# ShenhanQian/KGDet

Measured on AMD Instinct MI355X. Metric: training images/sec (whole node) KGDet R50-FPN 800x1333, higher is better.
Workload: dtype f32 (3 MFMA products per multiply on hi/lo-split operands -- fp16 parts forward, bf16 parts for gradients --, f32 accumulate); 1 GPU; KGDet R50-FPN train step, 2 img/GPU at 800x1333 (padded 800x1344), DeformConv fwd/bwd + focal/moment losses + grad-clip + Adam; no collective at dp1 (one rank: nothing to exchange); global_batch=2, parallelism=dp1

## Files before the change

### include/kgdet_hip.h

```cpp
#ifndef KGDET_HIP_H_
#define KGDET_HIP_H_

#include <stddef.h>
#include <stdint.h>

#ifdef __cplusplus
extern "C" {
#endif

#define KGDET_OK 0
#define KGDET_E_SHAPE 1
#define KGDET_E_WORKSPACE 2
#define KGDET_E_HIP 3
size_t kgdet_conv_packed_bytes(int32_t M, int32_t K, int32_t taps);
int kgdet_conv_pack(const float *w, int32_t O, int32_t C, int32_t taps, int32_t transpose, void *packed, void *stream);
int kgdet_conv_pack_fmt(const float *w, int32_t O, int32_t C, int32_t taps, int32_t transpose, void *packed,
                        int32_t operand_format, void *stream);
int kgdet_conv_pack_both_fmt(const float *w, int32_t O, int32_t C, int32_t taps, void *packed, void *packed_t,
                             int32_t forward_format, void *stream);
int kgdet_conv_apply_epilogue_fmt(const void *packed, const float *x, float *y, const float *bias, const float *residual,
                                  int32_t relu, int64_t B, int32_t M, int32_t K, int32_t H, int32_t W, int32_t taps,
                                  int32_t stride, int32_t operand_format, void *workspace, size_t workspace_bytes,
                                  void *stream);
int kgdet_conv_apply_gated_fmt(const void *packed, const float *x, float *y, const float *bias, const float *residual,
                               int32_t relu, const float *gate, int64_t B, int32_t M, int32_t K, int32_t H, int32_t W,
                               int32_t taps, int32_t stride, int32_t operand_format, void *workspace, size_t workspace_bytes,
                               void *stream);
int kgdet_stem_conv7x7_s2_fmt(const void *packed, const float *x, float *y, int64_t B, int32_t H, int32_t W,
                              int32_t operand_format, void *stream);
int kgdet_conv_pack_both(const float *w, int32_t O, int32_t C, int32_t taps, void *packed, void *packed_t, void *stream);
int64_t kgdet_conv_pack_blocks(int32_t O, int32_t C, int32_t taps);
int kgdet_conv_pack_multi(const int64_t *desc_dev, int32_t n, int64_t total_blocks, void *stream);
size_t kgdet_conv_apply_workspace_bytes(int64_t B, int32_t M, int32_t K, int32_t H, int32_t W, int32_t taps,
                                        int32_t stride);
int kgdet_conv_apply(const void *packed, const float *x, float *y, int64_t B, int32_t M, int32_t K, int32_t H, int32_t W,
                     int32_t taps, int32_t stride, void *workspace, size_t workspace_bytes, void *stream);
#define KGDET_CONV_APPLY_PLAN_WORDS 11
int kgdet_conv_apply_plan(int64_t B, int32_t M, int32_t K, int32_t H, int32_t W, int32_t taps, int32_t stride,
                          int32_t out[KGDET_CONV_APPLY_PLAN_WORDS]);
int kgdet_conv_apply_epilogue(const void *packed, const float *x, float *y, const float *bias, const float *residual,
                              int32_t relu, int64_t B, int32_t M, int32_t K, int32_t H, int32_t W, int32_t taps,
                              int32_t stride, void *workspace, size_t workspace_bytes, void *stream);
int kgdet_stem_conv7x7_s2(const void *packed, const float *x, float *y, int64_t B, int32_t H, int32_t W, void *stream);
int kgdet_conv3x3_s2_grad_input(const void *packed_t, const float *grad_y, float *grad_x, int64_t B, int32_t C, int32_t O,
                                int32_t Hin, int32_t Win, void *stream);
size_t kgdet_conv3x3_s2_grad_weight_workspace_bytes(int64_t B, int32_t O, int32_t C, int32_t H, int32_t W);
int kgdet_conv3x3_s2_grad_weight(const float *grad_y, const float *x, float *grad_w, int64_t B, int32_t O, int32_t C, int32_t H,
                                 int32_t W, void *workspace, size_t workspace_bytes, void *stream);
size_t kgdet_conv1x1_grad_weight_workspace_bytes(int64_t B, int32_t O, int32_t C, int64_t HW);
int kgdet_conv1x1_grad_weight(const float *grad_y, const float *x, float *grad_w, int64_t B, int32_t O, int32_t C,
                              int64_t HW, void *workspace, size_t workspace_bytes, void *stream);
size_t kgdet_conv3x3_grad_weight_workspace_bytes(int64_t B, int32_t O, int32_t C, int32_t H, int32_t W);
int kgdet_conv3x3_grad_weight(const float *grad_y, const float *x, float *grad_w, int64_t B, int32_t O, int32_t C,
                              int32_t H, int32_t W, void *workspace, size_t workspace_bytes, void *stream);
#define KGDET_CONV_GRAD_WEIGHT_PLAN_WORDS 10
int kgdet_conv_grad_weight_plan(int64_t B, int32_t O, int32_t C, int32_t H, int64_t W, int32_t taps,
                                int32_t out[KGDET_CONV_GRAD_WEIGHT_PLAN_WORDS]);

int kgdet_bn_act_forward(const float *x, const float *gamma, const float *beta, const float *mean, const float *var,
                         float eps, const float *residual, float *y, int64_t N, int32_t C, int64_t HW, int32_t relu,
                         void *stream);
int32_t kgdet_bn_act_partials(int64_t N, int32_t C, int64_t HW);
int kgdet_bn_act_backward(const float *grad_y, const float *x, const float *y, const float *gamma, const float *beta,
                          const float *mean, const float *var, float eps, int32_t has_residual, int32_t relu,
                          float *grad_x, float *grad_residual, float *partial, float *sums, int64_t N, int32_t C,
                          int64_t HW, void *stream);
int kgdet_conv1x1_nhwc_residual(const void *x, const void *weight, const float *bias, const void *residual, void *out,
                                int64_t M, int32_t K, int32_t N, int32_t relu, void *stream);
int kgdet_conv1x1_nhwc_residual_in(const void *x, const float *in_bias, const void *weight, const float *bias,
                                   const void *residual, void *out, int64_t M, int32_t K, int32_t N, int32_t relu,
                                   void *stream);
int kgdet_bn_fold_backward(const float *grad_z, const float *z, int32_t relu, float *g, float *partial, int64_t N, int32_t C,
                           int64_t HW, void *stream);
int kgdet_bn_fold_finish(const float *partial, int32_t P, const float *w, float *G , const float *s,
                         const float *mean, const float *var, float eps, float *grad_beta ,
                         float *grad_gamma , int32_t O, int32_t CK, void *stream);
int kgdet_conv1x1_grad_weight_fold(const float *grad_y, const float *x, float *grad_w, int64_t B, int32_t O, int32_t C,
                                   int64_t HW, void *workspace, size_t workspace_bytes, const float *w, const float *s,
                                   const float *mean, const float *var, float eps, const float *bn_partial, int32_t P,
                                   float *grad_beta , float *grad_gamma , void *stream);
int kgdet_conv3x3_grad_weight_fold(const float *grad_y, const float *x, float *grad_w, int64_t B, int32_t O, int32_t C,
                                   int32_t H, int32_t W, void *workspace, size_t workspace_bytes, const float *w,
                                   const float *s, const float *mean, const float *var, float eps, const float *bn_partial,
                                   int32_t P, float *grad_beta , float *grad_gamma , void *stream);
int kgdet_bn_relu_maxpool(const float *x, const float *gamma, const float *beta, const float *mean, const float *var,
                          float eps, float *y, int64_t N, int32_t C, int32_t H, int32_t W, void *stream);

int kgdet_bias_act(void *x, const float *bias, const void *residual, int64_t N, int32_t C, int64_t HW, int32_t dtype,
                   int32_t relu, int32_t channels_last, void *stream);
int kgdet_bias_relu_maxpool_nhwc(const void *x, const float *bias, void *y, int64_t N, int32_t C, int32_t H, int32_t W,
                                 int32_t dtype, void *stream);

#define KGDET_E_UNSUPPORTED 4
#define KGDET_E_PARTIAL 5

const char *kgdet_last_error(void);
int kgdet_version(void);
int kgdet_device_cu_count(void);

#define KGDET_OPT_EXACT_BACKWARD 0
#define KGDET_OPT_FWD_COLUMN_WAVE 1
#define KGDET_OPT_WGRAD_STREAMK 2
#define KGDET_OPT_BWD_PHASE 3
#define KGDET_OPT_COUNT 4
int kgdet_set_option(int32_t option, int32_t value);

typedef struct kgdet_dcn_shape {
  int32_t N, C, H, W;
  int32_t O, kh, kw;
  int32_t stride_h, stride_w, pad_h, pad_w, dil_h, dil_w;
  int32_t groups, deformable_groups;
  int32_t out_channel_offset, out_channels_total;
} kgdet_dcn_shape;

#define KGDET_DCN_RELU 1u
#define KGDET_DCN_BF16 2u
#define KGDET_DCN_EXACT_FP32 4u

int kgdet_dcn_output_size(const kgdet_dcn_shape *s, int32_t *Ho, int32_t *Wo);

size_t kgdet_dcn_packed_weight_bytes(const kgdet_dcn_shape *s);
size_t kgdet_dcn_workspace_bytes(const kgdet_dcn_shape *s);

int kgdet_dcn_pack_weight(const kgdet_dcn_shape *s, const float *weight, float *packed, void *stream);
int kgdet_dcn_pack_weight_multi(int32_t n, const kgdet_dcn_shape *const *shapes, const float *const *weights,
                                float *const *packeds, void *stream);
int kgdet_dcn_pack_weight_images(int32_t n, const kgdet_dcn_shape *const *shapes, const float *const *weights,
                                 float *const *packeds, uint32_t images, void *stream);
int32_t kgdet_dcn_split_path_complete(const kgdet_dcn_shape *shape);
int kgdet_dcn_unpack_weight_grad(const kgdet_dcn_shape *s, const float *packed, float *grad_weight,
                                 int accumulate, void *stream);

int kgdet_deform_conv_forward(const kgdet_dcn_shape *s, const float *input, const float *offset,
                              const float *mask , const float *packed_weight,
                              const float *bias , float *output, uint32_t flags,
                              void *workspace, size_t workspace_bytes, void *stream);

size_t kgdet_dcn_group_workspace_bytes(int32_t n, const kgdet_dcn_shape *const *shapes);

int kgdet_deform_conv_forward_grouped(int32_t n, const kgdet_dcn_shape *const *shapes, const float *const *inputs,
                                      const float *const *offsets, const float *const *masks ,
                                      const float *const *packed_weights, const float *const *biases ,
                                      float *const *outputs, uint32_t flags, void *workspace,
                                      size_t workspace_bytes, void *stream);

int kgdet_deform_conv_grad_input(const kgdet_dcn_shape *s, const float *offset, const float *mask ,
                                 const float *packed_weight, const float *grad_output, float *grad_input,
                                 uint32_t flags, void *workspace, size_t workspace_bytes, void *stream);

int kgdet_deform_conv_grad_offset(const kgdet_dcn_shape *s, const float *input, const float *offset,
                                  const float *packed_weight, const float *grad_output, float *grad_offset,
                                  uint32_t flags, void *workspace, size_t workspace_bytes, void *stream);

int kgdet_deform_conv_backward_input_grouped(int32_t n, const kgdet_dcn_shape *const *shapes, const float *const *inputs,
                                             const float *const *offsets, const float *const *packed_weights,
                                             const float *const *grad_outputs, float *const *grad_inputs,
                                             float *const *grad_offsets, void *workspace, size_t workspace_bytes,
                                             void *stream);

int kgdet_deform_conv_grad_weight_grouped(int32_t n, const kgdet_dcn_shape *const *shapes, const float *const *inputs,
                                          const float *const *offsets, const float *const *grad_outputs,
                                          float *const *grad_weights, void *workspace, size_t workspace_bytes,
                                          void *stream);

int kgdet_deform_conv_backward_input(const kgdet_dcn_shape *s, const float *input, const float *offset,
                                     const float *mask , const float *packed_weight,
                                     const float *grad_output, float *grad_input, float *grad_offset,
                                     float *grad_mask , void *workspace,
                                     size_t workspace_bytes, void *stream);

int kgdet_deform_conv_backward_weight(const kgdet_dcn_shape *s, const float *input, const float *offset,
                                      const float *mask , const float *grad_output,
                                      float *grad_weight, float *grad_bias , int accumulate,
                                      void *workspace, size_t workspace_bytes, void *stream);

typedef struct kgdet_psroi_shape {
  int32_t B, C, H, W;
  int32_t R;
  int32_t out_dim, group_size, pooled_size, part_size, sample_per_part;
  int32_t no_trans, num_classes;
  float spatial_scale, trans_std;
} kgdet_psroi_shape;

size_t kgdet_deform_psroi_forward_workspace_bytes(const kgdet_psroi_shape *s);
int kgdet_deform_psroi_forward(const kgdet_psroi_shape *s, const float *data, const float *rois,
                               const float *trans, float *out, float *count, void *workspace, size_t workspace_bytes,
                               void *stream);
// ... 275 lines not shown
```

### kgdet_amd/_lib.py

```python
import ctypes
import os
import subprocess

_HERE = os.path.dirname(os.path.abspath(__file__))
LIB_PATH = os.environ.get('KGDET_LIB') or os.path.join(_HERE, 'libkgdet_hip.so')
CSRC = os.path.join(_HERE, 'csrc')

KGDET_OK = 0
KGDET_E_SHAPE = 1
KGDET_E_WORKSPACE = 2
KGDET_E_HIP = 3
KGDET_E_UNSUPPORTED = 4
KGDET_E_PARTIAL = 5

DCN_RELU = 1
DCN_BF16 = 2
DCN_EXACT_FP32 = 4


class DcnShape(ctypes.Structure):
    _fields_ = [(n, ctypes.c_int32) for n in (
        'N', 'C', 'H', 'W', 'O', 'kh', 'kw', 'stride_h', 'stride_w', 'pad_h', 'pad_w', 'dil_h',
        'dil_w', 'groups', 'deformable_groups', 'out_channel_offset', 'out_channels_total')]


class PsroiShape(ctypes.Structure):
    _fields_ = [(n, ctypes.c_int32) for n in (
        'B', 'C', 'H', 'W', 'R', 'out_dim', 'group_size', 'pooled_size', 'part_size',
        'sample_per_part', 'no_trans', 'num_classes')] + [
        ('spatial_scale', ctypes.c_float), ('trans_std', ctypes.c_float)]


class AugSegment(ctypes.Structure):
    _fields_ = [('boxes', ctypes.c_void_p), ('scores', ctypes.c_void_p), ('kpts', ctypes.c_void_p), ('n', ctypes.c_int64),
                ('img_w', ctypes.c_float), ('scale', ctypes.c_double), ('flip', ctypes.c_int32)]


PREPROC_MAX_JOBS = 32
COCO_ACC_TILE = 1024
COCO_PACK_ROWS = 4
COCO_ORDER_MAX_ROWS = 1024
COCO_ORDER_MAX_LABELS = 64
COCO_JSON_MAX_K = 1024
DRAW_MAX_IMAGES, DRAW_MAX_ROWS, DRAW_MAX_K, DRAW_MAX_LABELS = 32, 1024, 1024, 64


class CocoPackedDets(ctypes.Structure):
    _fields_ = [('n', ctypes.c_int64)] + [(n, ctypes.c_void_p) for n in (
        'cell', 'img_idx', 'cat_idx', 'id', 'score', 'bbox', 'area', 'kxy32')]


class PreprocJob(ctypes.Structure):
    _fields_ = [('src', ctypes.c_void_p), ('src_h', ctypes.c_int32), ('src_w', ctypes.c_int32),
                ('src_row_bytes', ctypes.c_int32), ('dst', ctypes.c_void_p), ('dst_channel_stride', ctypes.c_int64),
                ('dst_row_stride', ctypes.c_int32), ('new_h', ctypes.c_int32), ('new_w', ctypes.c_int32),
                ('out_h', ctypes.c_int32), ('out_w', ctypes.c_int32), ('scale_y', ctypes.c_float),
                ('scale_x', ctypes.c_float), ('flip', ctypes.c_int32)]


PREPROC_AUG_MAX_JOBS = 16
AUG_COLOUR, AUG_BRIGHTNESS, AUG_CONTRAST, AUG_CONTRAST_FIRST, AUG_SATURATION, AUG_HUE, AUG_PERMUTE = 1, 2, 4, 8, 16, 32, 64


class PreprocAugJob(ctypes.Structure):
    _fields_ = PreprocJob._fields_ + [
        ('vh', ctypes.c_int32), ('vw', ctypes.c_int32), ('oy', ctypes.c_int32), ('ox', ctypes.c_int32),
        ('fill', ctypes.c_float * 3), ('delta', ctypes.c_float), ('alpha', ctypes.c_float), ('sat', ctypes.c_float),
        ('hue', ctypes.c_float), ('perm', ctypes.c_int32), ('flags', ctypes.c_uint32)]


def build(force=False):
    cmd = ['make', '-C', CSRC, '-j8']
    if force:
        cmd.append('-B')
    subprocess.check_call(cmd)
    return LIB_PATH


_lib = None


def lib():
    global _lib
    if _lib is None:
        if not os.path.exists(LIB_PATH):
            raise ImportError(
                'kgdet_amd: %s is missing -- run `python -c "import __graft_entry__ as g; g.build()"` '
                'or `make -C kgdet_amd/csrc`. There is no non-HIP fallback.' % LIB_PATH)
        L = ctypes.CDLL(LIB_PATH)
        L.kgdet_last_error.restype = ctypes.c_char_p
        for name in ('kgdet_dcn_packed_weight_bytes', 'kgdet_dcn_workspace_bytes', 'kgdet_dcn_group_workspace_bytes',
                     'kgdet_nms_workspace_bytes', 'kgdet_deform_psroi_backward_workspace_bytes',
                     'kgdet_deform_psroi_forward_workspace_bytes', 'kgdet_head_loss_workspace_bytes', 'kgdet_serial_loss_workspace_bytes',
                     'kgdet_moment_bbox_backward_workspace_bytes', 'kgdet_multiclass_soft_nms_workspace_bytes'):
            if hasattr(L, name):
                getattr(L, name).restype = ctypes.c_size_t
        for name in ('kgdet_multiclass_soft_nms_supported', 'kgdet_multiclass_nms_supported'):
            if hasattr(L, name):
                getattr(L, name).restype = ctypes.c_int
                getattr(L, name).argtypes = [ctypes.c_int32] * 4
        if hasattr(L, 'kgdet_coco_similarity'):
            vp, i32, i64 = ctypes.c_void_p, ctypes.c_int32, ctypes.c_int64
            L.kgdet_coco_similarity.restype = L.kgdet_coco_match.restype = ctypes.c_int
            L.kgdet_coco_similarity.argtypes = [i32, vp, vp, i32, i64, i64, i64] + [vp] * 8 + [i32, vp, vp]
            L.kgdet_coco_match.argtypes = [vp, vp, i32, i64, i64, i64] + [vp] * 6 + [i32, vp, i32] + [vp] * 5
        if hasattr(L, 'kgdet_coco_accumulate'):
            vp, i32, i64 = ctypes.c_void_p, ctypes.c_int32, ctypes.c_int64
            L.kgdet_coco_count_gt.restype = L.kgdet_coco_accumulate.restype = L.kgdet_coco_pack_landmarks.restype = ctypes.c_int
            L.kgdet_coco_count_gt.argtypes = [vp, vp, i64, i32, i32, vp, vp]
            L.kgdet_coco_accumulate.argtypes = [vp] * 9 + [i64] + [i32] * 5 + [i64] + [vp] * 4 + [ctypes.c_size_t, vp]
            L.kgdet_coco_pack_landmarks.argtypes = [vp, i64, i32, i32, vp, vp, vp, vp]
        if hasattr(L, 'kgdet_coco_order_dets'):
            vp, i32, i64 = ctypes.c_void_p, ctypes.c_int32, ctypes.c_int64
            L.kgdet_coco_order_dets.restype = L.kgdet_coco_scatter_dets.restype = ctypes.c_int
            L.kgdet_coco_order_dets.argtypes = [vp, i64, i32, i32, vp, vp, i32, i32, i64, i32, i32, i32] + [vp] * 7
            L.kgdet_coco_scatter_dets.argtypes = ([vp, i64, i32, i32, vp, i32, i64] + [vp] * 5 + [i32, i32]
                                                  + [ctypes.POINTER(CocoPackedDets)] * 2 + [vp, vp])
        if hasattr(L, 'kgdet_coco_json_write'):
            vp, i32, i64 = ctypes.c_void_p, ctypes.c_int32, ctypes.c_int64
            L.kgdet_coco_json_measure.restype = L.kgdet_coco_json_write.restype = ctypes.c_int
            L.kgdet_coco_json_measure.argtypes = [vp, i64, i32, i32] + [vp] * 5 + [i32, i32, vp, vp, vp, i64, vp, vp]
            L.kgdet_coco_json_write.argtypes = [i32, vp, i64, i32, i32] + [vp] * 5 + [i32, i32, i64, i64, i64, vp, i64, vp, vp]
        if hasattr(L, 'kgdet_draw_detections'):
            vp, i32, i64 = ctypes.c_void_p, ctypes.c_int32, ctypes.c_int64
            L.kgdet_draw_detections.restype = ctypes.c_int
            L.kgdet_draw_detections.argtypes = ([vp, i64, vp, i64, vp, vp, i32, vp, i64, i32, i32, vp, i32, vp, vp, i32, vp, vp,
                                                 ctypes.c_float] + [i32] * 6 + [vp])
        _lib = L
    return _lib


def check(rc, what=''):
    if rc == KGDET_OK:
        return
    msg = lib().kgdet_last_error().decode('utf-8', 'replace')
    if rc == KGDET_E_UNSUPPORTED:
        raise NotImplementedError('%s: %s' % (what, msg))
    raise RuntimeError('%s: %s' % (what, msg))


def ptr(t):
    return ctypes.c_void_p(t.data_ptr()) if t is not None else ctypes.c_void_p(0)


def raw_stream(device_index=None):
    import torch
    if device_index is None:
        device_index = torch.cuda.current_device()
    return torch._C._cuda_getCurrentRawStream(device_index)


def current_stream():
    return ctypes.c_void_p(raw_stream())
```

### kgdet_amd/csrc/dense_forward.hip

```cpp
#include "dense_common.h"

namespace kgdet {

__global__ __launch_bounds__(256) void conv1x1_pack(const float *__restrict__ w, int O, int C, int T, int transpose,
                                                    unsigned char *__restrict__ img, unsigned char *__restrict__ img_t,
                                                    int f16_forward) {
  if (gridDim.y == 2) {
    transpose = blockIdx.y;
    img = blockIdx.y ? img_t : img;
  }
  const bool f16 = f16_forward && !transpose;
  f16_saturate_on();
  const int M = transpose ? C : O, K = transpose ? O : C;
  const int k16s = (K + kTK - 1) / kTK;
  const long long total = (long long)((M + kTM - 1) / kTM) * k16s * T * 2 * kTM;
  for (long long i = blockIdx.x * 256LL + threadIdx.x; i < total; i += gridDim.x * 256LL) {
    const int row = (int)(i % kTM);
    const int khalf = (int)((i / kTM) & 1);
    const long long st = i / (2 * kTM);
    const int t = (int)(st % T);
    const int k16 = (int)((st / T) % k16s), mt = (int)(st / ((long long)T * k16s));
    const int m = mt * kTM + row, k0 = k16 * kTK + khalf * 8;
    float v[8];
#pragma unroll
// ... 189 lines not shown
#pragma unroll
    for (int mi = 0; mi < 2; ++mi) {
      acc[mi] = mfma_t<F16>(a[1][mi], bb[0], acc[mi]);
      acc[mi] = mfma_t<F16>(a[0][mi], bb[1], acc[mi]);
      acc[mi] = mfma_t<F16>(a[0][mi], bb[0], acc[mi]);
    }
  };
  {
    Regs R[kPF];
#pragma unroll
    for (int i = 0; i < kPF; ++i) issue(i, R[i]);
    commit(0, R[0]);
    const int full = stages / kPF * kPF;
    for (int s0 = 0; s0 < full; s0 += kPF) {
#pragma unroll
      for (int u = 0; u < kPF; ++u) {
        const int s = s0 + u;
        __syncthreads();
        issue(s + kPF, R[u]);
        multiply(s & 1);
        commit((s + 1) & 1, R[(u + 1) % kPF]);
      }
    }
#pragma unroll
    for (int u = 0; u < kPF - 1; ++u) {
      const int s = full + u;
      if (s < stages) {
        __syncthreads();
        multiply(s & 1);
        if (s + 1 < stages) commit((s + 1) & 1, R[u + 1]);
      }
    }
  }

  float *yb = y + (long long)part * part_stride + (long long)b * M * N;
  const int n = n0 + wn * 32 + (lane & 31);
  if constexpr (F16) {
#pragma unroll
    for (int mi = 0; mi < 2; ++mi)
#pragma unroll
      for (int r = 0; r < 16; ++r) acc[mi][r] *= 1.0f / kF16WeightScale;
  }
  if (bias || residual) {
    const int nc = min(n, N - 1);
    float add[2][16];
#pragma unroll
    for (int mi = 0; mi < 2; ++mi)
#pragma unroll
      for (int r = 0; r < 16; ++r) {
        const int m = min(mt * kTM + wm * 64 + mi * 32 + (r & 3) + 8 * (r >> 2) + 4 * (lane >> 5), M - 1);
        float v = bias ? bias[m] : 0.0f;
        if (residual) v += residual[((long long)b * M + m) * N + nc];
        add[mi][r] = v;
      }
#pragma unroll
    for (int mi = 0; mi < 2; ++mi)
#pragma unroll
      for (int r = 0; r < 16; ++r) acc[mi][r] += add[mi][r];
  }
  if (gate) {
    const int nc = min(n, N - 1);
    float gv[2][16];
#pragma unroll
    for (int mi = 0; mi < 2; ++mi)
#pragma unroll
      for (int r = 0; r < 16; ++r) {
        const int m = min(mt * kTM + wm * 64 + mi * 32 + (r & 3) + 8 * (r >> 2) + 4 * (lane >> 5), M - 1);
        gv[mi][r] = gate[((long long)b * M + m) * N + nc];
      }
#pragma unroll
    for (int mi = 0; mi < 2; ++mi)
#pragma unroll
      for (int r = 0; r < 16; ++r) acc[mi][r] = gv[mi][r] > 0.0f ? acc[mi][r] : 0.0f;
  }
#pragma unroll
  for (int mi = 0; mi < 2; ++mi)
#pragma unroll
    for (int r = 0; r < 16; ++r) {
      const int m = mt * kTM + wm * 64 + mi * 32 + (r & 3) + 8 * (r >> 2) + 4 * (lane >> 5);
      if (m < M && n < N) yb[(long long)m * N + n] = relu ? fmaxf(acc[mi][r], 0.0f) : acc[mi][r];
    }
}

constexpr int kPatchMax = 256;
constexpr int kPatchPart = 2 * kPatchMax * 16;
constexpr int kPatchBuf = 2 * kPatchPart;
template <int WAVES, int NB, bool F16 = false>
__global__ __launch_bounds__(64 * WAVES) void conv3x3_patch4(const unsigned char *__restrict__ img,
                                                             const float *__restrict__ x, float *__restrict__ y, int M,
                                                             int K, int H, int W, int n_mt, int tiles_x, int n_nt,
                                                             int tiles, int ksplit, long long part_stride, int TX, int TY,
                                                             const float *__restrict__ bias,
                                                             const float *__restrict__ residual, int relu,
    const float *__restrict__ gate = nullptr) {
  __shared__ __attribute__((aligned(16))) unsigned char smem[2 * kPatchBuf];
  if constexpr (F16) f16_saturate_on();
  constexpr int HALVES = 4 / WAVES, THREADS = 64 * WAVES, PXT = kPatchMax / THREADS;
  const int unit0 = xcd_tile(blockIdx.x, tiles * ksplit * HALVES);
  if (unit0 >= tiles * ksplit * HALVES) return;
  const int half = unit0 % HALVES, unit = unit0 / HALVES;
  const int part = unit % ksplit, tile = unit / ksplit;
  const int tid = threadIdx.x, lane = tid & 63, wave = (tid >> 6) + half * WAVES;
  const int N = H * W;
  const int chunks_all = K / kTK, per = (chunks_all + ksplit - 1) / ksplit;
  const int c_begin = part * per, c_end = max(c_begin, min(chunks_all, c_begin + per));
  const int chunks = c_end - c_begin, stages = chunks * 9;
  const int mt = tile % n_mt, nt = (tile / n_mt) % n_nt, b = tile / (n_mt * n_nt);
  const int y0 = (nt / tiles_x) * TY, x0 = (nt % tiles_x) * TX;
  const int PW = TX + 2, PP = PW * (TY + 2);

  if (mt * kTM + half * 64 >= M) return;
  bool p_live[PXT];
  int p_off[PXT];
#pragma unroll
  for (int i = 0; i < PXT; ++i) {
    const int pp = tid + i * THREADS;
    const int ppy = pp / PW, ppx = pp - ppy * PW;
    const int iy = y0 - 1 + ppy, ix = x0 - 1 + ppx;
    p_live[i] = pp < PP && iy >= 0 && iy < H && ix >= 0 && ix < W;
    p_off[i] = p_live[i] ? iy * W + ix : 0;
  }
  const float *xb = x + (long long)b * K * N;
  unsigned char *b_dst = smem + tid * 16;

  int b_rd[NB], o_n[NB];
  bool o_live[NB];
#pragma unroll
  for (int nb = 0; nb < NB; ++nb) {
    const int qq = nb * 32 + (lane & 31), q = min(qq, TX * TY - 1);
    const int py = q / TX, px = q - py * TX;
    b_rd[nb] = ((lane >> 5) * kPatchMax + py * PW + px) * 16;
    o_live[nb] = qq < TX * TY && y0 + py < H && x0 + px < W;
    o_n[nb] = o_live[nb] ? (y0 + py) * W + x0 + px : 0;
  }
  const int row_pitch = PW * 16;
  const unsigned char *ag = img + ((long long)mt * chunks_all + min(c_begin, chunks_all - 1)) * 9 * kStage +
                            (lane >> 5) * (kTM * 16) + (wave * 32 + (lane & 31)) * 16;

  f32x16 acc[NB];
#pragma unroll
  for (int i = 0; i < NB; ++i)
#pragma unroll
    for (int r = 0; r < 16; ++r) acc[i][r] = 0.0f;

  float bv[PXT][16];
  auto issue_b = [&](int ci) {
    const float *xp = xb + (long long)min(c_begin + min(ci, chunks - 1), chunks_all - 1) * kTK * N;
#pragma unroll
    for (int i = 0; i < PXT; ++i)
#pragma unroll
      for (int j = 0; j < 16; ++j) bv[i][j] = xp[(long long)j * N + p_off[i]];
  };
  auto commit_b = [&](int buf) {
#pragma unroll
    for (int i = 0; i < PXT; ++i)
#pragma unroll
      for (int j = 0; j < 16; ++j) asm volatile("" : "+v"(bv[i][j]));
#pragma unroll
    for (int i = 0; i < PXT; ++i)
#pragma unroll
      for (int kh = 0; kh < 2; ++kh) {
        float v[8];
#pragma unroll
        for (int j = 0; j < 8; ++j) v[j] = p_live[i] ? bv[i][kh * 8 + j] : 0.0f;
        bf16x8 hi, lo;
        split8_t<F16>(v, hi, lo);
// ... 305 lines not shown
  return ((t0 > t1 ? t0 : t1) + 255) / 256;
}

template <typename Kernel, typename... Args>
void launch_fmt(bool f16, Kernel bf16_kernel, Kernel f16_kernel, unsigned grid, unsigned block, void *stream, Args... args) {
  hipLaunchKernelGGL(f16 ? f16_kernel : bf16_kernel, dim3(grid), dim3(block), 0, (hipStream_t)stream, args...);
}

int nn_ksplit(long long tiles, int stages) {
  if (tiles >= 200) return 1;
  int k = (int)((384 + tiles - 1) / tiles);
  const int most = stages / 8;
  if (k > most) k = most;
  if (k > 8) k = 8;
  return k < 1 ? 1 : k;
}

struct NNPlan {
  bool patch, halves;
  int TX, TY, NB, NW, tiles_x, n_nt, ks;
  long long tiles;
};
NNPlan plan_nn(long long B, int M, int K, int H, int W, int taps, int stride) {
  NNPlan p;
  const int Ho = (H + stride - 1) / stride, Wo = (W + stride - 1) / stride;
  const int n_mt = (M + kTM - 1) / kTM;
  p.patch = taps == 9 && stride == 1;
  p.TX = p.TY = p.tiles_x = 0;
  p.NB = p.NW = 4;
  p.n_nt = (int)(((long long)Ho * Wo + kTN - 1) / kTN);
  if (p.patch) {
    long long best = -1;
    for (int cap = 128; cap <= (M > 64 ? 160 : 128); cap += 32)
      for (int tx = 8; tx <= 126 && tx <= (W + 7) / 8 * 8; ++tx) {
        const int ty = cap / tx;
        if (ty < 1 || (tx + 2) * (ty + 2) > kPatchMax) continue;
        const long long n = (long long)((H + ty - 1) / ty) * ((W + tx - 1) / tx);
        const long long units = n * n_mt * B;
        const long long rounds = units <= 256 ? 256 : units <= 512 ? 512 : units;
        const long long cost = (rounds * (cap / 32)) * 4096 + n * 8 + (cap == 160) * 4 + ((tx + 2) * (ty + 2) > 230);
        if (best < 0 || cost < best) { best = cost; p.TX = tx; p.TY = ty; p.NB = cap / 32; }
      }
    static const int force_tx = env_int("KGDET_CONV_TX", 0);
    if (force_tx > 0 && (force_tx + 2) * (128 / force_tx + 2) <= kPatchMax) { p.TX = force_tx; p.TY = 128 / force_tx; p.NB = 4; }
    p.tiles_x = (W + p.TX - 1) / p.TX;
    p.n_nt = p.tiles_x * ((H + p.TY - 1) / p.TY);
  } else {
    static const int force_nw = env_int("KGDET_CONV_NW", 0);
    const long long hw = (long long)Ho * Wo;
    const long long u4 = (long long)n_mt * ((hw + 127) / 128) * B, u5 = (long long)n_mt * ((hw + 159) / 160) * B;
    const long long c4 = ((u4 + 255) / 256) * 4, c5 = ((u5 + 255) / 256) * 5;
    if (force_nw == 5 || (force_nw == 0 && u4 >= 200 && u5 >= 200 && c5 * 10 <= c4 * 9)) {
      p.NW = 5;
      p.n_nt = (int)((hw + 159) / 160);
    }
  }
  p.tiles = (long long)n_mt * p.n_nt * B;
  p.ks = nn_ksplit(p.tiles, taps * ((K + kTK - 1) / kTK));
  if (p.patch && p.tiles < 200) {
    const int chunks = K / kTK;
    double best = 1e30;
    p.ks = 1;
    for (int ks = 1; ks <= 8 && ks * 2 <= chunks; ++ks) {
      const double out_mb = (double)B * M * Ho * Wo * 4e-6;
      const double cost = (double)((p.tiles * ks + 255) / 256) * ((chunks + ks - 1) / ks) + 0.114 * out_mb * ks;
      if (cost < best) { best = cost; p.ks = ks; }
    }
  }
  static const int force_ks = env_int("KGDET_CONV_KS", 0);
  if (force_ks > 0) p.ks = force_ks;
  static const int force_halves = env_int("KGDET_CONV_HALVES", -1);
  p.halves = p.patch && p.NB == 4 &&
             (force_halves >= 0 ? force_halves != 0 : ((p.ks == 1 && p.tiles > 256 && p.tiles < 400) || M <= 64));
  return p;
}

enum NNCloser { kCloseStore = 0, kCloseSumEpilogue = 1, kCloseSumBiasAct = 2, kCloseSum = 3 };
NNCloser nn_closer(int ks, long long HW, bool epilogue) {
  if (ks <= 1) return kCloseStore;
  if (!epilogue) return kCloseSum;
  return HW % 2 == 0 ? kCloseSumEpilogue : kCloseSumBiasAct;
}

}

}

using namespace kgdet;

extern "C" size_t kgdet_conv_packed_bytes(int32_t M, int32_t K, int32_t taps) {
  if (M <= 0 || K <= 0 || (taps == 9 && K % kTK) || (taps != 1 && taps != 9)) return 0;
  return (size_t)pack_items(M, K, taps) * 32;
}

extern "C" int kgdet_conv_pack_fmt(const float *w, int32_t O, int32_t C, int32_t taps, int32_t transpose, void *packed,
                                   int32_t operand_format, void *stream) {
  const int M = transpose ? C : O, K = transpose ? O : C;
  KGDET_CHECK_SHAPE(taps == 1 || taps == 9, "taps must be 1 (1x1) or 9 (3x3)");
  KGDET_CHECK_SHAPE(O > 0 && C > 0 && (taps == 1 || K % kTK == 0), "reduction length %d is not a multiple of 16", K);
  KGDET_CHECK_SHAPE(w && packed, "null pointer");
  const long long blocks = (pack_items(M, K, taps) + 255) / 256;
  hipLaunchKernelGGL(conv1x1_pack, dim3((unsigned)(blocks > 65535 ? 65535 : blocks)), dim3(256), 0, (hipStream_t)stream, w,
                     O, C, taps, transpose, (unsigned char *)packed, (unsigned char *)nullptr, operand_format == 1 ? 1 : 0);
  KGDET_CHECK_LAUNCH("conv_pack");
  return KGDET_OK;
}

extern "C" int kgdet_conv_pack(const float *w, int32_t O, int32_t C, int32_t taps, int32_t transpose, void *packed,
                               void *stream) {
  return kgdet_conv_pack_fmt(w, O, C, taps, transpose, packed, 0, stream);
}

extern "C" int kgdet_conv_pack_both_fmt(const float *w, int32_t O, int32_t C, int32_t taps, void *packed, void *packed_t,
                                        int32_t forward_format, void *stream) {
  KGDET_CHECK_SHAPE(taps == 1 || taps == 9, "taps must be 1 (1x1) or 9 (3x3)");
  KGDET_CHECK_SHAPE(O > 0 && C > 0 && (taps == 1 || (O % kTK == 0 && C % kTK == 0)), "O and C must be multiples of 16");
  KGDET_CHECK_SHAPE(w && packed && packed_t, "null pointer");
  const long long blocks = pack_both_blocks(O, C, taps);
  hipLaunchKernelGGL(conv1x1_pack, dim3((unsigned)(blocks > 32768 ? 32768 : blocks), 2), dim3(256), 0,
                     (hipStream_t)stream, w, O, C, taps, 0, (unsigned char *)packed, (unsigned char *)packed_t,
                     forward_format == 1 ? 1 : 0);
  KGDET_CHECK_LAUNCH("conv_pack_both");
  return KGDET_OK;
}

extern "C" int kgdet_conv_pack_both(const float *w, int32_t O, int32_t C, int32_t taps, void *packed, void *packed_t,
                                    void *stream) {
  return kgdet_conv_pack_both_fmt(w, O, C, taps, packed, packed_t, 0, stream);
}

extern "C" int64_t kgdet_conv_pack_blocks(int32_t O, int32_t C, int32_t taps) {
  if (O <= 0 || C <= 0 || (taps == 9 && (O % kTK || C % kTK)) || (taps != 1 && taps != 9)) return 0;
  return pack_both_blocks(O, C, taps);
}

extern "C" int kgdet_conv_pack_multi(const int64_t *desc_dev, int32_t n, int64_t total_blocks, void *stream) {
  KGDET_CHECK_SHAPE(desc_dev && n > 0 && total_blocks > 0 && total_blocks < (1LL << 31), "bad descriptor table");
  hipLaunchKernelGGL(conv1x1_pack_multi, dim3((unsigned)total_blocks), dim3(256), 0, (hipStream_t)stream,
                     (const long long *)desc_dev, n);
  KGDET_CHECK_LAUNCH("conv_pack_multi");
  return KGDET_OK;
}

extern "C" size_t kgdet_conv_apply_workspace_bytes(int64_t B, int32_t M, int32_t K, int32_t H, int32_t W,
                                                    int32_t taps, int32_t stride) {
  if (B <= 0 || M <= 0 || K <= 0 || H <= 0 || W <= 0 || (taps == 9 && K % kTK) || stride < 1 || stride > 2) return 0;
  const long long HW = (long long)((H + stride - 1) / stride) * ((W + stride - 1) / stride);
  const int ks = plan_nn(B, M, K, H, W, taps, stride).ks;
  return ks > 1 ? (size_t)ks * B * M * HW * sizeof(float) : 0;
}

extern "C" int kgdet_conv_apply_plan(int64_t B, int32_t M, int32_t K, int32_t H, int32_t W, int32_t taps, int32_t stride,
                                     int32_t out[KGDET_CONV_APPLY_PLAN_WORDS]) {
  KGDET_CHECK_SHAPE(out, "null pointer");
  KGDET_CHECK_SHAPE(B > 0 && M > 0 && K > 0 && H > 0 && W > 0 && (long long)H * W < (1LL << 30), "bad sizes");
  KGDET_CHECK_SHAPE(taps == 1 || taps == 9, "taps must be 1 (1x1) or 9 (3x3)");
  KGDET_CHECK_SHAPE(stride == 1 || stride == 2, "stride must be 1 or 2");
  KGDET_CHECK_SHAPE(taps == 1 || K % kTK == 0, "reduction length %d is not a multiple of 16", K);
  const NNPlan p = plan_nn(B, M, K, H, W, taps, stride);
  KGDET_CHECK_SHAPE(p.tiles < (1LL << 28), "too many tiles");
  const long long HW = (long long)((H + stride - 1) / stride) * ((W + stride - 1) / stride);
  const int32_t words[KGDET_CONV_APPLY_PLAN_WORDS] = {
      p.patch, p.TX, p.TY, p.NB, p.NW, p.ks, p.halves, (int32_t)p.tiles, p.n_nt, nn_closer(p.ks, HW, true), nn_closer(p.ks, HW, false)};
  for (int i = 0; i < KGDET_CONV_APPLY_PLAN_WORDS; ++i) out[i] = words[i];
  return KGDET_OK;
}

extern "C" int kgdet_conv_apply_epilogue_fmt(const void *packed, const float *x, float *y, const float *bias,
                                             const float *residual, int32_t relu, int64_t B, int32_t M, int32_t K,
                                             int32_t H, int32_t W, int32_t taps, int32_t stride, int32_t operand_format,
                                             void *workspace, size_t workspace_bytes, void *stream) {
  return kgdet_conv_apply_gated_fmt(packed, x, y, bias, residual, relu, nullptr, B, M, K, H, W, taps, stride, operand_format,
                                    workspace, workspace_bytes, stream);
}

extern "C" int kgdet_conv_apply_gated_fmt(const void *packed, const float *x, float *y, const float *bias,
                                          const float *residual, int32_t relu, const float *gate, int64_t B, int32_t M,
                                          int32_t K, int32_t H, int32_t W, int32_t taps, int32_t stride,
                                          int32_t operand_format, void *workspace, size_t workspace_bytes, void *stream) {
  const bool f16 = operand_format == 1;
  KGDET_CHECK_SHAPE(B >= 0 && M > 0 && K > 0 && H >= 0 && W >= 0 && (long long)H * W < (1LL << 30), "bad sizes");
  KGDET_CHECK_SHAPE(taps == 1 || taps == 9, "taps must be 1 (1x1) or 9 (3x3)");
  KGDET_CHECK_SHAPE(stride == 1 || stride == 2, "stride must be 1 or 2");
  KGDET_CHECK_SHAPE(taps == 1 || K % kTK == 0, "reduction length %d is not a multiple of 16", K);
  const int Ho = (H + stride - 1) / stride, Wo = (W + stride - 1) / stride;
  const long long HW = (long long)Ho * Wo;
  if (B * HW == 0) return KGDET_OK;
  KGDET_CHECK_SHAPE(packed && x && y, "null pointer");
  const NNPlan plan = plan_nn(B, M, K, H, W, taps, stride);
  const int n_mt = (M + kTM - 1) / kTM, n_nt = plan.n_nt;
  const long long tiles = plan.tiles;
  KGDET_CHECK_SHAPE(tiles < (1LL << 28), "too many tiles");
  const int ks = plan.ks;
  const long long part_stride = B * M * HW;
  if (ks > 1) {
    KGDET_CHECK_SHAPE(workspace && workspace_bytes >= (size_t)ks * part_stride * sizeof(float), "workspace too small");
    KGDET_CHECK_SHAPE(part_stride % 2 == 0, "B*M*Ho*Wo must be even");
    KGDET_CHECK_SHAPE(!gate || HW % 2 == 0, "a gated K-split convolution needs an even pixel count");
  }
  const unsigned grid = (unsigned)((tiles * ks + 7) / 8) * 8;
  float *dst = ks > 1 ? (float *)workspace : y;
  const float *k_bias = ks > 1 ? nullptr : bias, *k_residual = ks > 1 ? nullptr : residual, *k_gate = ks > 1 ? nullptr : gate;
  const int k_relu = ks > 1 ? 0 : relu;
  const unsigned char *img = (const unsigned char *)packed;
  if (plan.patch) {
    auto launch = [&](auto bf16_kernel, auto f16_kernel, unsigned g, unsigned threads) {
      launch_fmt(f16, bf16_kernel, f16_kernel, g, threads, stream, img, x, dst, M, K, H, W, n_mt, plan.tiles_x, n_nt, (int)tiles,
                 ks, part_stride, plan.TX, plan.TY, k_bias, k_residual, k_relu, k_gate);
    };
    if (plan.NB == 5)
      launch(conv3x3_patch4<4, 5, false>, conv3x3_patch4<4, 5, true>, grid, 256);
    else if (plan.halves)
      launch(conv3x3_patch4<2, 4, false>, conv3x3_patch4<2, 4, true>, (unsigned)((tiles * ks * 2 + 7) / 8) * 8, 128);
    else
      launch(conv3x3_patch4<4, 4, false>, conv3x3_patch4<4, 4, true>, grid, 256);
  } else {
    auto launch = [&](auto bf16_kernel, auto f16_kernel, unsigned threads) {
      launch_fmt(f16, bf16_kernel, f16_kernel, grid, threads, stream, img, x, dst, M, K, Ho, Wo, n_mt, n_nt, (int)tiles, ks,
                 part_stride, H, W, stride, k_bias, k_residual, k_relu, k_gate);
    };
    if (taps == 1 && plan.NW == 5)
      launch(conv_nn<1, 5, false>, conv_nn<1, 5, true>, 640);
    else if (taps == 1)
      launch(conv_nn<1, 4, false>, conv_nn<1, 4, true>, 512);
    else if (plan.NW == 5)
      launch(conv_nn<9, 5, false>, conv_nn<9, 5, true>, 640);
    else
      launch(conv_nn<9, 4, false>, conv_nn<9, 4, true>, 512);
  }
  KGDET_CHECK_LAUNCH("conv_nn");
  if (ks > 1) {
    const long long blocks = (part_stride / 2 + 255) / 256;
    const NNCloser closer = nn_closer(ks, HW, bias || residual || relu || gate);
    if (closer == kCloseSumEpilogue)
      hipLaunchKernelGGL(conv1x1_sum_epilogue, dim3((unsigned)(blocks > 2048 ? 2048 : blocks)), dim3(256), 0,
                         (hipStream_t)stream, (const float *)workspace, y, part_stride, part_stride, ks, bias, residual, relu,
                         M, (long long)HW, gate);
    else
      hipLaunchKernelGGL(conv1x1_sum, dim3((unsigned)(blocks > 2048 ? 2048 : blocks)), dim3(256), 0, (hipStream_t)stream,
                         (const float *)workspace, y, part_stride, part_stride, ks);
    KGDET_CHECK_LAUNCH("conv1x1_sum");
    if (closer == kCloseSumBiasAct) return kgdet_bias_act(y, bias, residual, B, M, HW, 0, relu, 0, stream);
  }
  return KGDET_OK;
}

extern "C" int kgdet_conv_apply_epilogue(const void *packed, const float *x, float *y, const float *bias,
                                         const float *residual, int32_t relu, int64_t B, int32_t M, int32_t K,
                                         int32_t H, int32_t W, int32_t taps, int32_t stride, void *workspace,
                                         size_t workspace_bytes, void *stream) {
  return kgdet_conv_apply_epilogue_fmt(packed, x, y, bias, residual, relu, B, M, K, H, W, taps, stride, 0, workspace,
                                       workspace_bytes, stream);
}

extern "C" int kgdet_conv3x3_s2_grad_input(const void *packed_t, const float *grad_y, float *grad_x, int64_t B, int32_t C,
                                           int32_t O, int32_t Hin, int32_t Win, void *stream) {
  KGDET_CHECK_SHAPE(B >= 0 && C > 0 && O > 0 && Hin > 0 && Win > 0 && O % kTK == 0, "bad sizes (O must be a multiple of 16)");
  if (B == 0) return KGDET_OK;
  KGDET_CHECK_SHAPE(packed_t && grad_y && grad_x, "null pointer");
  const int H = (Hin + 1) / 2, W = (Win + 1) / 2;
  int TX = 0, TY = 0;
  long long best = -1;
  for (int tx = 8; tx <= 64; ++tx) {
    const int ty = 64 / tx;
    if (ty < 1 || (tx + 2) * (ty + 2) > kPatchMax) continue;
    const long long n = (long long)((H + ty - 1) / ty) * ((W + tx - 1) / tx);
    const long long cost = n * 1024 + (tx + 2) * (ty + 2);
    if (best < 0 || cost < best) { best = cost; TX = tx; TY = ty; }
  }
  const int n_mt = (C + kTM - 1) / kTM, tiles_x = (W + TX - 1) / TX, n_nt = tiles_x * ((H + TY - 1) / TY);
  const long long tiles = (long long)n_mt * n_nt * B;
  KGDET_CHECK_SHAPE(tiles < (1LL << 28), "too many tiles");
  hipLaunchKernelGGL(conv3x3_s2_grad_input, dim3((unsigned)((tiles + 7) / 8 * 8)), dim3(256), 0, (hipStream_t)stream,
                     (const unsigned char *)packed_t, grad_y, grad_x, C, O, H, W, Hin, Win, n_mt, tiles_x, n_nt, (int)tiles, TX, TY);
  KGDET_CHECK_LAUNCH("conv3x3_s2_grad_input");
  return KGDET_OK;
}

extern "C" int kgdet_stem_conv7x7_s2_fmt(const void *packed, const float *x, float *y, int64_t B, int32_t H, int32_t W,
                                         int32_t operand_format, void *stream) {
  KGDET_CHECK_SHAPE(B >= 0 && H > 0 && W > 0, "bad sizes");
  if (B == 0) return KGDET_OK;
  KGDET_CHECK_SHAPE(packed && x && y, "null pointer");
  const int Ho = (H - 1) / 2 + 1, Wo = (W - 1) / 2 + 1;
  const int tiles_x = (Wo + kStemTX - 1) / kStemTX, tiles_per_image = tiles_x * ((Ho + kStemTY - 1) / kStemTY);
  KGDET_CHECK_SHAPE((long long)B * tiles_per_image < (1LL << 31), "too many tiles");
  launch_fmt(operand_format == 1, stem_conv7x7_s2<false>, stem_conv7x7_s2<true>, (unsigned)(B * tiles_per_image), 256, stream,
             (const unsigned char *)packed, x, y, H, W, Ho, Wo, tiles_x, tiles_per_image);
// ... 16 lines not shown
```

Measured before the change: 189.1 img/s.

## Add LDS-resident activation-row kernel for 1x1 stride-1 convolutions

Adds a new 1x1 conv forward kernel in which each 512-thread workgroup loads a 128-pixel column strip of the input for its whole K-range into LDS once, split into hi/lo parts. It then loops over several M tiles (MG output-channel tiles, two wavegroups), reusing the staged activations while streaming the packed weights through a register prefetch ring. A planner enables it by default for large, non-K-split 1x1 convs with K between 64 and 256, and an option can disable or force it. The goal is to stop re-reading and re-splitting activations for every M tile, at the cost of up to 128 KB of LDS per workgroup and fewer resident workgroups.

```diff
diff --git a/include/kgdet_hip.h b/include/kgdet_hip.h
--- a/include/kgdet_hip.h
+++ b/include/kgdet_hip.h
@@ -38,6 +38,9 @@
 #define KGDET_CONV_APPLY_PLAN_WORDS 11
 int kgdet_conv_apply_plan(int64_t B, int32_t M, int32_t K, int32_t H, int32_t W, int32_t taps, int32_t stride,
                           int32_t out[KGDET_CONV_APPLY_PLAN_WORDS]);
+#define KGDET_CONV_ROWS_PLAN_WORDS 5
+int kgdet_conv_apply_rows_plan(int64_t B, int32_t M, int32_t K, int32_t H, int32_t W, int32_t taps, int32_t stride,
+                               int32_t out[KGDET_CONV_ROWS_PLAN_WORDS]);
 int kgdet_conv_apply_epilogue(const void *packed, const float *x, float *y, const float *bias, const float *residual,
                               int32_t relu, int64_t B, int32_t M, int32_t K, int32_t H, int32_t W, int32_t taps,
                               int32_t stride, void *workspace, size_t workspace_bytes, void *stream);
@@ -102,7 +105,8 @@
 #define KGDET_OPT_FWD_COLUMN_WAVE 1
 #define KGDET_OPT_WGRAD_STREAMK 2
 #define KGDET_OPT_BWD_PHASE 3
-#define KGDET_OPT_COUNT 4
+#define KGDET_OPT_CONV_ROWS 4
+#define KGDET_OPT_COUNT 5
 int kgdet_set_option(int32_t option, int32_t value);
 
 typedef struct kgdet_dcn_shape {
diff --git a/kgdet_amd/_lib.py b/kgdet_amd/_lib.py
--- a/kgdet_amd/_lib.py
+++ b/kgdet_amd/_lib.py
@@ -16,6 +16,8 @@
 DCN_RELU = 1
 DCN_BF16 = 2
 DCN_EXACT_FP32 = 4
+OPT_CONV_ROWS = 4
+CONV_ROWS_PLAN_WORDS = 5
 
 
 class DcnShape(ctypes.Structure):
@@ -99,6 +101,9 @@
             if hasattr(L, name):
                 getattr(L, name).restype = ctypes.c_int
                 getattr(L, name).argtypes = [ctypes.c_int32] * 4
+        if hasattr(L, 'kgdet_conv_apply_rows_plan'):
+            L.kgdet_conv_apply_rows_plan.restype = ctypes.c_int
+            L.kgdet_conv_apply_rows_plan.argtypes = [ctypes.c_int64] + [ctypes.c_int32] * 6 + [ctypes.c_void_p]
         if hasattr(L, 'kgdet_coco_similarity'):
             vp, i32, i64 = ctypes.c_void_p, ctypes.c_int32, ctypes.c_int64
             L.kgdet_coco_similarity.restype = L.kgdet_coco_match.restype = ctypes.c_int
diff --git a/kgdet_amd/csrc/dense_forward.hip b/kgdet_amd/csrc/dense_forward.hip
--- a/kgdet_amd/csrc/dense_forward.hip
+++ b/kgdet_amd/csrc/dense_forward.hip
@@ -295,6 +295,175 @@
     }
 }
 
+constexpr int kRowsPF = 4;
+constexpr int kRowsLdsMax = 128 * 1024;
+template <int NW, bool F16>
+__global__ __launch_bounds__(512) void conv_nn_rows(const unsigned char *__restrict__ img, const float *__restrict__ x,
+                                                    float *__restrict__ y, int M, int K, int N, int n_mt, int n_nt, int MG,
+                                                    int units, int ksplit, long long part_stride,
+                                                    const float *__restrict__ bias, const float *__restrict__ residual,
+                                                    int relu, const float *__restrict__ gate) {
+  constexpr int TN = 32 * NW, kChunk = 4 * TN * 16, kPartB = 2 * TN * 16;
+  extern __shared__ __attribute__((aligned(16))) unsigned char rows_smem[];
+  if constexpr (F16) f16_saturate_on();
+  const int unit = xcd_tile(blockIdx.x, units);
+  if (unit >= units) return;
+  const int n_g = (n_mt + MG - 1) / MG;
+  const int part = unit % ksplit, g = (unit / ksplit) % n_g, nt = (unit / (ksplit * n_g)) % n_nt, b = unit / (ksplit * n_g * n_nt);
+  const int tid = threadIdx.x, lane = tid & 63, w = (tid >> 6) & 3, wg = tid >> 8;
+  const int S = K / kTK, per = (S + ksplit - 1) / ksplit;
+  const int s_begin = part * per, s_end = max(s_begin, min(S, s_begin + per));
+  const int stages = s_end - s_begin;
+  const int n0 = nt * TN;
+
+  const int mt_first = g * MG + wg, mt_end = min(g * MG + MG, n_mt);
+  const unsigned char *a_lane = img + (lane >> 5) * (kTM * 16) + (w * 32 + (lane & 31)) * 16;
+  const bool roll = stages % kRowsPF == 0;
+  auto issue_a = [&](int mt, int s, bf16x8 (&r)[2]) {
+    if (s >= stages) {
+      mt = roll ? mt + 2 : mt;
+      s = roll ? s - stages : stages - 1;
+    }
+    const unsigned char *p = a_lane + ((long long)min(mt, n_mt - 1) * S + min(s_begin + max(min(s, stages - 1), 0), S - 1)) * kStage;
+    r[0] = *reinterpret_cast<const bf16x8 *>(p);
+    r[1] = *reinterpret_cast<const bf16x8 *>(p + kPart);
+  };
+  bf16x8 AR[kRowsPF][2];
+#pragma unroll
+  for (int j = 0; j < kRowsPF; ++j) issue_a(mt_first, j, AR[j]);
+
+  {
+    const float *xb = x + ((long long)b * K + (long long)s_begin * kTK) * N;
+    const int items = stages * 2 * TN;
+    for (int i0 = 0; i0 < items; i0 += 1024) {
+      float v[2][8];
+      int n[2], ck[2];
+#pragma unroll
+      for (int e = 0; e < 2; ++e) {
+        const int it = min(i0 + e * 512 + tid, items - 1);
+        ck[e] = it / TN;
+        n[e] = it - ck[e] * TN;
+        const float *xp = xb + (long long)ck[e] * 8 * N + min(n0 + n[e], N - 1);
+#pragma unroll
+        for (int j = 0; j < 8; ++j) v[e][j] = xp[(long long)j * N];
+      }
+#pragma unroll
+      for (int e = 0; e < 2; ++e) {
+        bf16x8 hi, lo;
+        split8_t<F16>(v[e], hi, lo);
+        if (i0 + e * 512 + tid < items) {
+          unsigned char *d = rows_smem + (ck[e] >> 1) * kChunk + (ck[e] & 1) * (TN * 16) + n[e] * 16;
+          *reinterpret_cast<bf16x8 *>(d) = hi;
+          *reinterpret_cast<bf16x8 *>(d + kPartB) = lo;
+        }
+      }
+    }
+  }
+  __syncthreads();
+
+  const unsigned char *b_lane = rows_smem + (lane >> 5) * (TN * 16) + (lane & 31) * 16;
+  f32x16 acc[NW];
+  auto multiply = [&](int s, const bf16x8 (&a)[2]) {
+    const unsigned char *bt = b_lane + s * kChunk;
+    bf16x8 bf[NW][2];
+#pragma unroll
+    for (int nb = 0; nb < NW; ++nb) {
+      bf[nb][0] = *reinterpret_cast<const bf16x8 *>(bt + nb * 512);
+      bf[nb][1] = *reinterpret_cast<const bf16x8 *>(bt + nb * 512 + kPartB);
+    }
+#pragma unroll
+    for (int nb = 0; nb < NW; ++nb) acc[nb] = mfma_t<F16>(a[1], bf[nb][0], acc[nb]);
+#pragma unroll
+    for (int nb = 0; nb < NW; ++nb) acc[nb] = mfma_t<F16>(a[0], bf[nb][1], acc[nb]);
+#pragma unroll
+    for (int nb = 0; nb < NW; ++nb) acc[nb] = mfma_t<F16>(a[0], bf[nb][0], acc[nb]);
+  };
+  const int full = stages / kRowsPF * kRowsPF;
+  const int nl = lane & 31;
+  int nc = nl;
+  auto e_col = [&](int nb) { return min(n0 + nb * 32 + nc, N - 1); };
+  for (int mt = mt_first; mt < mt_end; mt += 2) {
+    const int m0 = mt * kTM + w * 32 + 4 * (lane >> 5);
+    constexpr int EB = NW;
+    float bv[16], pre[NW][16];
+    asm volatile("" : "+v"(nc));
+    int mr = m0;
+    auto e_row = [&](int r) { return ((long long)b * M + min(mr + (r & 3) + 8 * (r >> 2), M - 1)) * N; };
+    const float *first = residual ? residual : gate;
+    if (first) {
+#pragma unroll
+      for (int nb = 0; nb < EB; ++nb)
+#pragma unroll
+        for (int r = 0; r < 16; ++r) pre[nb][r] = first[e_row(r) + e_col(nb)];
+    }
+#pragma unroll
+    for (int nb = 0; nb < NW; ++nb)
+#pragma unroll
+      for (int r = 0; r < 16; ++r) acc[nb][r] = 0.0f;
+    for (int s0 = 0; s0 < full; s0 += kRowsPF) {
+#pragma unroll
+      for (int u = 0; u < kRowsPF; ++u) {
+        multiply(s0 + u, AR[u]);
+        __builtin_amdgcn_sched_barrier(0);
+        issue_a(mt, s0 + u + kRowsPF, AR[u]);
+        __builtin_amdgcn_sched_barrier(0);
+      }
+    }
+    if (!roll) {
+#pragma unroll
+      for (int u = 0; u < kRowsPF - 1; ++u)
+        if (full + u < stages) multiply(full + u, AR[u]);
+#pragma unroll
+      for (int j = 0; j < kRowsPF; ++j) issue_a(mt + 2, j, AR[j]);
+    }
+
+    float *yb = y + (long long)part * part_stride + (long long)b * M * N;
+    asm volatile("" : "+v"(mr), "+v"(nc));
+#pragma unroll
+    for (int r = 0; r < 16; ++r) bv[r] = bias ? bias[min(mr + (r & 3) + 8 * (r >> 2), M - 1)] : 0.0f;
+    if (first) {
+#pragma unroll
+      for (int nb = EB; nb < NW; ++nb)
+#pragma unroll
+        for (int r = 0; r < 16; ++r) pre[nb][r] = first[e_row(r) + e_col(nb)];
+    }
+#pragma unroll
+    for (int nb = 0; nb < NW; ++nb) {
+      if constexpr (F16) {
+#pragma unroll
+        for (int r = 0; r < 16; ++r) acc[nb][r] *= 1.0f / kF16WeightScale;
+      }
+      if (bias || residual) {
+#pragma unroll
+        for (int r = 0; r < 16; ++r) {
+          float v = bias ? bv[r] : 0.0f;
+          if (residual) v += pre[nb][r];
+          acc[nb][r] += v;
+        }
+      }
+    }
+    if (gate && residual) {
+#pragma unroll
+      for (int nb = 0; nb < NW; ++nb)
+#pragma unroll
+        for (int r = 0; r < 16; ++r) pre[nb][r] = gate[e_row(r) + e_col(nb)];
+    }
+#pragma unroll
+    for (int nb = 0; nb < NW; ++nb) {
+      const int n = n0 + nb * 32 + nc;
+      if (gate) {
+#pragma unroll
+        for (int r = 0; r < 16; ++r) acc[nb][r] = pre[nb][r] > 0.0f ? acc[nb][r] : 0.0f;
+      }
+#pragma unroll
+      for (int r = 0; r < 16; ++r) {
+        const int m = mr + (r & 3) + 8 * (r >> 2);
+        if (m < M && n < N) yb[(long long)m * N + n] = relu ? fmaxf(acc[nb][r], 0.0f) : acc[nb][r];
+      }
+    }
+  }
+}
+
 constexpr int kPatchMax = 256;
 constexpr int kPatchPart = 2 * kPatchMax * 16;
 constexpr int kPatchBuf = 2 * kPatchPart;
@@ -766,6 +935,35 @@
   return HW % 2 == 0 ? kCloseSumEpilogue : kCloseSumBiasAct;
 }
 
+struct RowsPlan {
+  bool taken;
+  int MG, NW, n_nt, lds;
+  long long wgs;
+};
+RowsPlan plan_rows(long long B, int M, int K, int H, int W, int taps, int stride, const NNPlan &p) {
+  RowsPlan r = {false, 0, 0, 0, 0, 0};
+  const int mode = g_options[KGDET_OPT_CONV_ROWS];
+  const int n_mt = (M + kTM - 1) / kTM;
+  const long long hw = (long long)H * W;
+  if (mode == 1 || taps != 1 || stride != 1 || n_mt < 2 || K % kTK || K < 64 || K > 256) return r;
+  const bool one_round = B * ((hw + 127) / 128) * ((n_mt + 1) / 2) * p.ks <= 256;
+  if (mode != 2 && (p.tiles < 200 || p.ks != 1 || one_round)) return r;
+  long long best = -1;
+  for (int nw = 4; nw >= 4; --nw) {
+    if ((long long)K * 32 * nw * 4 > kRowsLdsMax) continue;
+    const int n_nt = (int)((hw + 32 * nw - 1) / (32 * nw));
+    for (int mg = 8; mg >= 2; mg >>= 1) {
+      if (mg > 2 && mg > n_mt) continue;
+      const long long wgs = B * n_nt * ((n_mt + mg - 1) / mg) * p.ks;
+      const long long cost = one_round ? (long long)nw * (16 - mg) : ((wgs + 255) / 256) * (mg < n_mt ? mg : n_mt) * nw;
+      if (best < 0 || cost < best) { best = cost; r.MG = mg; r.NW = nw; r.n_nt = n_nt; r.wgs = wgs; }
+    }
+  }
+  r.lds = ((K / kTK + p.ks - 1) / p.ks) * 4 * 32 * r.NW * 16;
+  r.taken = true;
+  return r;
+}
+
 }
 
 }
@@ -847,6 +1045,24 @@
   const int32_t words[KGDET_CONV_APPLY_PLAN_WORDS] = {
       p.patch, p.TX, p.TY, p.NB, p.NW, p.ks, p.halves, (int32_t)p.tiles, p.n_nt, nn_closer(p.ks, HW, true), nn_closer(p.ks, HW, false)};
   for (int i = 0; i < KGDET_CONV_APPLY_PLAN_WORDS; ++i) out[i] = words[i];
+  return KGDET_OK;
+}
+
+extern "C" int kgdet_conv_apply_rows_plan(int64_t B, int32_t M, int32_t K, int32_t H, int32_t W, int32_t taps, int32_t stride,
+                                          int32_t out[KGDET_CONV_ROWS_PLAN_WORDS]) {
+  KGDET_CHECK_SHAPE(out, "null pointer");
+  KGDET_CHECK_SHAPE(B >= 0 && M > 0 && K > 0 && H >= 0 && W >= 0 && (long long)H * W < (1LL << 30), "bad sizes");
+  KGDET_CHECK_SHAPE(taps == 1 || taps == 9, "taps must be 1 (1x1) or 9 (3x3)");
+  KGDET_CHECK_SHAPE(stride == 1 || stride == 2, "stride must be 1 or 2");
+  KGDET_CHECK_SHAPE(taps == 1 || K % kTK == 0, "reduction length %d is not a multiple of 16", K);
+  RowsPlan r = {false, 0, 0, 0, 0, 0};
+  if (B * H * W != 0) {
+    const NNPlan p = plan_nn(B, M, K, H, W, taps, stride);
+    KGDET_CHECK_SHAPE(p.tiles < (1LL << 28), "too many tiles");
+    r = plan_rows(B, M, K, H, W, taps, stride, p);
+  }
+  const int32_t words[KGDET_CONV_ROWS_PLAN_WORDS] = {r.taken, r.MG, 32 * r.NW, (int32_t)r.wgs, r.lds};
+  for (int i = 0; i < KGDET_CONV_ROWS_PLAN_WORDS; ++i) out[i] = words[i];
   return KGDET_OK;
 }
 
@@ -887,7 +1103,17 @@
   const float *k_bias = ks > 1 ? nullptr : bias, *k_residual = ks > 1 ? nullptr : residual, *k_gate = ks > 1 ? nullptr : gate;
   const int k_relu = ks > 1 ? 0 : relu;
   const unsigned char *img = (const unsigned char *)packed;
-  if (plan.patch) {
+  const RowsPlan rows = plan_rows(B, M, K, H, W, taps, stride, plan);
+  if (rows.taken) {
+    KGDET_CHECK_SHAPE(rows.wgs < (1LL << 28), "too many tiles");
+    if (int rc = allow_lds<conv_nn_rows<4, false>, conv_nn_rows<4, true>>(kRowsLdsMax)) return rc;
+    auto launch = [&](auto bf16_kernel, auto f16_kernel) {
+      hipLaunchKernelGGL(f16 ? f16_kernel : bf16_kernel, dim3((unsigned)((rows.wgs + 7) / 8) * 8), dim3(512), (size_t)rows.lds,
+                         (hipStream_t)stream, img, x, dst, M, K, (int)HW, n_mt, rows.n_nt, rows.MG, (int)rows.wgs, ks, part_stride,
+                         k_bias, k_residual, k_relu, k_gate);
+    };
+    launch(conv_nn_rows<4, false>, conv_nn_rows<4, true>);
+  } else if (plan.patch) {
     auto launch = [&](auto bf16_kernel, auto f16_kernel, unsigned g, unsigned threads) {
       launch_fmt(f16, bf16_kernel, f16_kernel, g, threads, stream, img, x, dst, M, K, H, W, n_mt, plan.tiles_x, n_nt, (int)tiles,
                  ks, part_stride, plan.TX, plan.TY, k_bias, k_residual, k_relu, k_gate);
```

Result: faster. 195.7 img/s (median of 6 runs) (+3.5%).
